# meudnaes/VoronoiRT

Measured on AMD Instinct MI355X. Metric: formal-solve cell-updates/sec, higher is better.
Workload: dtype f64

## Files before the change

### include/voronoirt.h

```cpp
#ifndef VORONOIRT_H
#define VORONOIRT_H

#include <stdint.h>

#ifdef __cplusplus
extern "C" {
#endif

#define VRT_OK 0
#define VRT_EINVAL (-1)
#define VRT_EGRID (-2)
#define VRT_ENODEVICE (-3)
#define VRT_ENOMEM (-4)
#define VRT_EIO (-5)

typedef struct vrt_grid vrt_grid;
typedef struct vrt_plan vrt_plan;

#define VRT_ALPHA_SITE 0
#define VRT_ALPHA_SITE_LAM 1
#define VRT_ALPHA_ANGLE_SITE_LAM 2
#define VRT_ALPHA_ANGLE_NATIVE 3
#define VRT_ALPHA_SITE_LAM_NATIVE 4

// ... 79 lines not shown
int vrt_plan_execute_dev_f32(vrt_plan *p, int64_t nlam, int64_t ld, const float *dS,
                             const float *dalpha, int alpha_mode, const float *dI0_up,
                             const float *dI0_down, const double *weights_host, float *dJ,
                             float *dI_out, void *stream);
int vrt_plan_last_sweep_timing(const vrt_plan *p, double *ms, int64_t *launches);
int vrt_plan_check(vrt_plan *p);
int vrt_plan_last_path(const vrt_plan *p);
int vrt_plan_set_option(vrt_plan *p, const char *name, const char *value);
int vrt_grid_set_option(vrt_grid *g, const char *name, const char *value);

typedef struct vrt_schedule vrt_schedule;
int vrt_schedule_build(const vrt_grid *g, int dir, const int64_t *up, int n_sweeps, vrt_schedule **out);
int64_t vrt_schedule_num_nodes(const vrt_schedule *s);
int64_t vrt_schedule_num_levels(const vrt_schedule *s);
int vrt_schedule_get(const vrt_schedule *s, int64_t *site, int32_t *zflags, int64_t *level_off);
void vrt_schedule_destroy(vrt_schedule *s);
int vrt_layer_schedule(const vrt_grid *g, int dir, const int64_t *up, int n_sweeps, uint32_t *vis,
                       int32_t *nlev, int64_t *n_visits);
int vrt_layer_sorted_slots(const vrt_grid *g, int dir, const uint32_t *vis, int64_t *store, int64_t *self);

typedef struct vrt_patch_schedule vrt_patch_schedule;
int vrt_patch_schedule_build(const vrt_grid *g, int dir, const int64_t *up, int n_sweeps, int own_target,
                             int entry_cap, vrt_patch_schedule **out, int64_t counts[6]);
int vrt_patch_schedule_get(const vrt_patch_schedule *s, int32_t *layer_patch_off, int32_t *patch_own_lo,
                           int32_t *patch_own_cnt, int32_t *patch_nlev, int64_t *patch_ent_off,
                           int32_t *entry_pos, uint32_t *entry_vis, uint32_t *entry_loc);
int vrt_patch_schedule_get_deps(const vrt_patch_schedule *s, int64_t *dep_off, int32_t *dep_list);
int vrt_patch_schedule_get_layers(const vrt_patch_schedule *s, uint32_t *vis, int32_t *nlev, int64_t *n_visits);
void vrt_patch_schedule_destroy(vrt_patch_schedule *s);

int vrt_delaunay_up(vrt_grid *g, const double k[3], const double *S, const double *I0,
                    int64_t nI0, const double *alpha, int n_sweeps, double *I_out);
int vrt_delaunay_down(vrt_grid *g, const double k[3], const double *S, const double *I0,
                      int64_t nI0, const double *alpha, int n_sweeps, double *I_out);

#define VRT_METRIC_EUCLIDEAN   0
#define VRT_METRIC_PERIODIC_XY 1
#define VRT_RASTER_NEAREST     1
#define VRT_RASTER_INV_DIST2   2
int vrt_grid_nearest(vrt_grid *g, int64_t nq, const double *q_zxy, int metric, int k, int64_t *idx, double *dist);
int vrt_grid_to_raster_dev(vrt_grid *g, int64_t nz, int64_t nx, int64_t ny, const double *z, const double *x,
                           const double *y, int metric, int mode, int64_t nf, int64_t ld, const double *d_fields,
                           double *d_raster, void *stream);
int vrt_raster_to_grid_dev(vrt_grid *g, int64_t nz, int64_t nx, int64_t ny, const double *z, const double *x,
                           const double *y, int64_t nf, const double *d_raster, int64_t ld, double *d_fields,
                           void *stream);
// ... 135 lines not shown
```

### voronoirt_amd/_lib.py

```python
from __future__ import annotations

import ctypes
import os

HERE = os.path.dirname(os.path.abspath(__file__))
LIB_PATH = os.path.join(HERE, "libvrt_hip.so")
if os.environ.get("VRT_LIB_PATH"):
    LIB_PATH = os.environ["VRT_LIB_PATH"]

c_i64 = ctypes.c_int64
c_dbl = ctypes.c_double
p_i64 = ctypes.POINTER(ctypes.c_int64)
p_i32 = ctypes.POINTER(ctypes.c_int32)
p_dbl = ctypes.POINTER(ctypes.c_double)
p_int = ctypes.POINTER(ctypes.c_int)
vp = ctypes.c_void_p

VRT_OK, VRT_EINVAL, VRT_EGRID, VRT_ENODEVICE, VRT_ENOMEM, VRT_EIO = 0, -1, -2, -3, -4, -5
ALPHA_SITE, ALPHA_SITE_LAM, ALPHA_ANGLE_SITE_LAM, ALPHA_ANGLE_NATIVE, ALPHA_SITE_LAM_NATIVE = 0, 1, 2, 3, 4
METRIC_EUCLIDEAN, METRIC_PERIODIC_XY = 0, 1
RASTER_NEAREST, RASTER_INV_DIST2 = 1, 2

class LineCaseStruct(ctypes.Structure):
    _fields_ = [("nlam", c_i64), ("lambda_", p_dbl), ("blocks", c_i64 * 6), ("lambda0", c_dbl), ("c0", c_dbl),
# ... 75 lines not shown
                                              p_dbl, p_dbl, p_dbl, p_dbl]),
    "vrt_multi_lambda_create": (ctypes.c_int, [vp, ctypes.POINTER(LineCaseStruct), p_dbl, ctypes.POINTER(vp)]),
    "vrt_multi_lambda_iterate": (ctypes.c_int, [vp, p_dbl]),
    "vrt_multi_lambda_get": (ctypes.c_int, [vp, p_dbl, p_dbl, p_dbl, p_dbl, p_dbl]),
    "vrt_multi_lambda_destroy": (None, [vp]),
    "vrt_rates_populations_dev": (ctypes.c_int, [vp, c_i64, c_i64, p_dbl, p_i64, vp, p_dbl, c_dbl, c_dbl, vp, vp,
                                                 c_dbl, p_dbl, p_dbl, vp, vp, c_dbl, c_dbl, c_dbl, vp, vp, vp,
                                                 vp, vp]),
    "vrt_plan_last_sweep_timing": (ctypes.c_int, [vp, p_dbl, p_i64]),
    "vrt_plan_last_path": (ctypes.c_int, [vp]),
    "vrt_plan_set_option": (ctypes.c_int, [vp, ctypes.c_char_p, ctypes.c_char_p]),
    "vrt_grid_set_option": (ctypes.c_int, [vp, ctypes.c_char_p, ctypes.c_char_p]),
    "vrt_schedule_build": (ctypes.c_int, [vp, ctypes.c_int, p_i64, ctypes.c_int,
                                          ctypes.POINTER(vp)]),
    "vrt_schedule_num_nodes": (c_i64, [vp]),
    "vrt_schedule_num_levels": (c_i64, [vp]),
    "vrt_schedule_get": (ctypes.c_int, [vp, p_i64, p_i32, p_i64]),
    "vrt_schedule_destroy": (None, [vp]),
    "vrt_layer_schedule": (ctypes.c_int, [vp, ctypes.c_int, p_i64, ctypes.c_int,
                                          ctypes.POINTER(ctypes.c_uint32), p_i32, p_i64]),
    "vrt_layer_sorted_slots": (ctypes.c_int, [vp, ctypes.c_int, ctypes.POINTER(ctypes.c_uint32), p_i64, p_i64]),
    "vrt_patch_schedule_build": (ctypes.c_int, [vp, ctypes.c_int, p_i64, ctypes.c_int, ctypes.c_int, ctypes.c_int,
                                                ctypes.POINTER(vp), p_i64]),
    "vrt_patch_schedule_get": (ctypes.c_int, [vp, p_i32, p_i32, p_i32, p_i32, p_i64, p_i32,
                                              ctypes.POINTER(ctypes.c_uint32), ctypes.POINTER(ctypes.c_uint32)]),
    "vrt_patch_schedule_get_deps": (ctypes.c_int, [vp, p_i64, p_i32]),
    "vrt_patch_schedule_get_layers": (ctypes.c_int, [vp, ctypes.POINTER(ctypes.c_uint32), p_i32, p_i64]),
    "vrt_patch_schedule_destroy": (None, [vp]),
    "vrt_lambda_update_dev": (ctypes.c_int, [vp, c_i64, c_i64, vp, vp, vp, vp, vp, p_dbl, vp]),
    "vrt_short_characteristics": (ctypes.c_int, [c_i64, c_i64, c_i64, p_dbl, p_dbl, p_dbl, c_i64, p_dbl,
                                                 p_int, p_dbl, c_i64, p_dbl, c_i64, p_dbl, ctypes.c_int,
                                                 ctypes.c_int, p_dbl]),
    "vrt_regular_create": (ctypes.c_int, [c_i64, c_i64, c_i64, p_dbl, p_dbl, p_dbl, ctypes.c_int,
                                          ctypes.POINTER(vp)]),
    "vrt_regular_destroy": (None, [vp]),
    "vrt_regular_execute_dev": (ctypes.c_int, [vp, c_i64, p_dbl, p_int, vp, c_i64, vp, c_i64, c_i64, vp,
                                               ctypes.c_int, vp, vp]),
    "vrt_regular_last_solve_ms": (ctypes.c_int, [vp, p_dbl]),
    "vrt_synth_opacity_dev": (ctypes.c_int, [c_i64, c_i64, c_i64, p_dbl, c_i64, p_dbl, p_dbl, c_dbl, c_dbl, c_dbl, c_dbl,
                                             c_dbl, c_dbl, c_dbl, c_dbl, vp, vp, vp, vp, vp, vp, vp, vp, vp, vp]),
    "vrt_synth_opacity": (ctypes.c_int, [ctypes.c_int, c_i64, c_i64, c_i64, p_dbl, c_i64, p_dbl, p_dbl, c_dbl, c_dbl,
                                         c_dbl, c_dbl, c_dbl, c_dbl, c_dbl, c_dbl, p_dbl, p_dbl, p_dbl, p_dbl, p_dbl,
                                         p_dbl, p_dbl, p_dbl, p_dbl]),
    "vrt_regular_emergent_dev": (ctypes.c_int, [vp, p_dbl, c_i64, vp, vp, ctypes.c_int, vp, vp]),
    "vrt_top_intensity": (ctypes.c_int, [c_i64, c_i64, c_i64, p_dbl, p_dbl, p_dbl, p_dbl, c_i64, p_dbl, p_dbl,
                                         ctypes.c_int, ctypes.c_int, p_dbl]),
# ... 57 lines not shown
```

### voronoirt_amd/api.py

```python
from __future__ import annotations

import ctypes
import os
import re
import weakref

import numpy as np

from . import _lib
from ._lib import VrtError, check

QUADRATURE_DIR = os.path.join(os.path.dirname(os.path.abspath(__file__)), "quadratures")


def _d(a):
    return a.ctypes.data_as(_lib.p_dbl) if a is not None else None


def _i(a):
    return a.ctypes.data_as(_lib.p_i64) if a is not None else None


def _f64(a):
    return np.ascontiguousarray(a, dtype=np.float64)
# ... 456 lines not shown
        site = np.zeros(nn, dtype=np.int64)
        z = np.zeros(nn, dtype=np.int32)
        off = np.zeros(nl + 1, dtype=np.int64)
        check(L.vrt_schedule_get(h, _i(site), z.ctypes.data_as(_lib.p_i32), _i(off)))
    finally:
        L.vrt_schedule_destroy(h)
    return site, z, off


def build_layer_schedule(sites: VoronoiSites, dir: int, up, n_sweeps: int = 3):
    L = _lib.load()
    up = np.ascontiguousarray(up, dtype=np.int64)
    vis = np.zeros(sites.n, dtype=np.uint32)
    layers = sites.layers_up if dir > 0 else sites.layers_down
    nlev = np.zeros(layers.size, dtype=np.int32)
    nv = ctypes.c_int64()
    check(L.vrt_layer_schedule(sites.handle, int(dir), _i(up), int(n_sweeps),
                               vis.ctypes.data_as(ctypes.POINTER(ctypes.c_uint32)),
                               nlev.ctypes.data_as(_lib.p_i32), ctypes.byref(nv)))
    return vis, nlev, nv.value


def build_patch_schedule(sites: VoronoiSites, dir: int, up, n_sweeps: int = 3, own_target: int = 768,
                         entry_cap: int = 1024) -> dict:
    L = _lib.load()
    up = np.ascontiguousarray(up, dtype=np.int64)
    h = ctypes.c_void_p()
    cnt = np.zeros(6, dtype=np.int64)
    check(L.vrt_patch_schedule_build(sites.handle, int(dir), _i(up), int(n_sweeps), int(own_target), int(entry_cap),
                                     ctypes.byref(h), _i(cnt)))
    try:
        P, E = int(cnt[0]), int(cnt[1])
        out = {"layer_patch_off": np.zeros(int(cnt[5]), dtype=np.int32), "patch_own_lo": np.zeros(P, dtype=np.int32),
               "patch_own_cnt": np.zeros(P, dtype=np.int32), "patch_nlev": np.zeros(P, dtype=np.int32),
               "patch_ent_off": np.zeros(P + 1, dtype=np.int64), "entry_pos": np.zeros(E, dtype=np.int32),
               "entry_vis": np.zeros(E, dtype=np.uint32), "entry_loc": np.zeros(E, dtype=np.uint32)}
        u32 = ctypes.POINTER(ctypes.c_uint32)
        check(L.vrt_patch_schedule_get(h, out["layer_patch_off"].ctypes.data_as(_lib.p_i32),
                                       out["patch_own_lo"].ctypes.data_as(_lib.p_i32),
                                       out["patch_own_cnt"].ctypes.data_as(_lib.p_i32),
                                       out["patch_nlev"].ctypes.data_as(_lib.p_i32), _i(out["patch_ent_off"]),
                                       out["entry_pos"].ctypes.data_as(_lib.p_i32),
                                       out["entry_vis"].ctypes.data_as(u32), out["entry_loc"].ctypes.data_as(u32)))
        out["dep_off"] = np.zeros(P + 1, dtype=np.int64)
        check(L.vrt_patch_schedule_get_deps(h, _i(out["dep_off"]), None))
        out["dep_list"] = np.zeros(int(out["dep_off"][-1]), dtype=np.int32)
        check(L.vrt_patch_schedule_get_deps(h, None, out["dep_list"].ctypes.data_as(_lib.p_i32)))
        out["layer_vis"] = np.zeros(sites.n, dtype=np.uint32)
        out["layer_nlev"] = np.zeros((sites.layers_up if dir > 0 else sites.layers_down).size, dtype=np.int32)
        nv = ctypes.c_int64()
        check(L.vrt_patch_schedule_get_layers(h, out["layer_vis"].ctypes.data_as(u32),
                                              out["layer_nlev"].ctypes.data_as(_lib.p_i32), ctypes.byref(nv)))
        out["layer_visits"] = nv.value
# ... 617 lines not shown
```

### voronoirt_amd/csrc/vrt_api.cpp

```cpp
#include <algorithm>
#include <atomic>
#include <chrono>
#include <cmath>
#include <cstdio>
#include <cstdlib>
#include <cstring>
#include <new>
#include <thread>

#include "vrt_internal.h"

namespace vrt {

static thread_local std::string g_err;

void set_error(const std::string &msg) { g_err = msg; }
int fail(int code, const std::string &msg)
{
    g_err = msg;
    return code;
}

void tuning_from_env(Tuning &t)
{
    static const char *names[] = {"VRT_PATH", "VRT_STEP_K", "VRT_STEP_SINGLE", "VRT_STEP_PAIRS", "VRT_STEP_XCD",
                                  "VRT_STEP_STREAMS", "VRT_STEP_LEVEL_MAP", "VRT_STEP_GROUP_DIR", "VRT_TILE_WIDE",
                                  "VRT_TILE_PRE", "VRT_PATCH_K", "VRT_PATCH_NT", "VRT_PATCH_OWN",
                                  "VRT_PATCH_Q", "VRT_PATCH_TARGET", "VRT_PATCH_SPLIT", "VRT_PAIR_BLOCK", "VRT_PATCH_QUAD", "VRT_PATCH_LEAN", "VRT_PATCH_CHAIN", "VRT_CHAIN_PAIRS", "VRT_CHAIN_SPIN", "VRT_CHAIN_DATAFLAG", "VRT_CHAIN_STATIC", "VRT_LAMBDA_NATIVE", "VRT_DEBUG_FLAGS", "VRT_DEBUG_SKIP_LEVELS",
                                  "VRT_TILE_DEBUG"};
    for (const char *nm : names) {
        const char *e = std::getenv(nm);
        if (e && *e && tuning_set(t, nm, e, false) != VRT_OK) {
            static std::mutex mu;
            static std::vector<std::string> said;
            std::lock_guard<std::mutex> lock(mu);
            if (std::find(said.begin(), said.end(), std::string(nm)) == said.end()) {
                said.push_back(nm);
                std::fprintf(stderr, "[libvrt_hip] ignoring %s=%s: %s\n", nm, e, g_err.c_str());
            }
        }
    }
}

int tuning_set(Tuning &t, const char *name, const char *value, bool created)
{
    if (!name || !value) return fail(VRT_EINVAL, "NULL option name or value");
    const std::string nm(name), v(value);
    if (nm == "VRT_PATH") {
        static const char *paths[] = {"auto", "levels", "tiles", "steps", "patches"};
        for (int i = 0; i < 5; i++)
            if (v == paths[i]) { t.path = i; return VRT_OK; }
        if (v.empty()) { t.path = 0; return VRT_OK; }
        return fail(VRT_EINVAL, "VRT_PATH must be auto, levels, tiles, steps or patches");
    }
    char *end = nullptr;
    const long x = std::strtol(value, &end, 10);
    if (end == value || *end != 0) return fail(VRT_EINVAL, "option " + nm + " needs an integer value");
    struct { const char *name; int *field; long lo, hi; bool creation_only; } tab[] = {
        {"VRT_STEP_K", &t.step_K, 0, 18, false}, {"VRT_STEP_SINGLE", &t.step_single, 0, 1, false},
        {"VRT_STEP_PAIRS", &t.step_pairs, 0, 64, false}, {"VRT_STEP_XCD", &t.step_xcd, 0, 2, false},
        {"VRT_STEP_STREAMS", &t.step_streams, 1, 4, false}, {"VRT_STEP_LEVEL_MAP", &t.step_level_map, 0, 1, false},
        {"VRT_STEP_GROUP_DIR", &t.step_group_dir, 0, 1, false}, {"VRT_TILE_WIDE", &t.tile_wide, 0, 1, false},
        {"VRT_TILE_PRE", &t.tile_pre, 0, 1, false},
        {"VRT_PATCH_K", &t.patch_K, 1, 8, true}, {"VRT_PATCH_NT", &t.patch_NT, 64, 1024, true},
        {"VRT_PATCH_OWN", &t.patch_own, 0, 65535, true}, {"VRT_PATCH_Q", &t.patch_Q, 1, 4, false},
        {"VRT_PATCH_TARGET", &t.patch_target, 0, 1 << 20, false}, {"VRT_PATCH_SPLIT", &t.patch_split, 0, 4096, false}, {"VRT_PAIR_BLOCK", &t.pair_block, 1, 16, true},
        {"VRT_PATCH_QUAD", &t.patch_quad, 0, 1, true}, {"VRT_PATCH_LEAN", &t.patch_lean, 0, 1, false},
        {"VRT_PATCH_CHAIN", &t.patch_chain, 0, 2, false}, {"VRT_CHAIN_PAIRS", &t.chain_pairs, 1, 256, false},
        {"VRT_CHAIN_SPIN", &t.chain_spin, 1, 1 << 20, false}, {"VRT_CHAIN_DATAFLAG", &t.chain_dataflag, 0, 2, false},
        {"VRT_LAMBDA_NATIVE", &t.lambda_native, 0, 1, false}, {"VRT_CHAIN_STATIC", &t.chain_static, 0, 1, false}, {"VRT_DEBUG_FLAGS", &t.debug_flags, 0, 1 << 20, false},
        {"VRT_DEBUG_SKIP_LEVELS", &t.debug_skip_levels, 0, 1, false}, {"VRT_TILE_DEBUG", &t.tile_debug, 0, 1, false},
    };
    for (auto &o : tab)
        if (nm == o.name) {
            if (o.creation_only && created)
                return fail(VRT_EINVAL, "option " + nm + " shapes what plan creation builds: preset it in the environment");
            if (x < o.lo || x > o.hi) return fail(VRT_EINVAL, "option " + nm + " out of range");
            *o.field = (int)x;
            return VRT_OK;
        }
    return fail(VRT_EINVAL, "unknown option " + nm);
}

template <typename T>
static int dev_alloc(T **p, size_t count)
{
    *p = nullptr;
    if (count == 0) count = 1;
// ... 376 lines not shown
            p->tune.patch_K = 1; p->tune.patch_NT = 512; p->tune.patch_Q = 1;
        }
        p->patch_K = p->tune.patch_K;
        p->patch_NT = p->tune.patch_NT;
        p->patch_cap = p->patch_K * p->patch_NT;
        int lg = 0;
        while ((2 << lg) <= p->tune.pair_block && lg < 4) lg++;
        while (lg > 0 && ((uint64_t)n << (lg + 4)) > 0xFFFFFFFFull) lg--;
        p->lg_pair_block = lg;
    }
    const int patch_own = p->tune.patch_own > 0 ? std::min(p->tune.patch_own, p->patch_cap) : p->patch_cap;
    {
        const unsigned hw = std::max(1u, std::thread::hardware_concurrency());
        const int nthr = std::max(1, (int)std::min<unsigned>(std::min(hw, (unsigned)A * 4u <= hw ? 64u : 16u), (unsigned)A));
        const int sub_threads = (int)std::max(1u, std::min(16u, hw / (unsigned)nthr));
        std::atomic<int> next_job(0);
        if (!run_workers(nthr, [&](int) {
                for (;;) {
                    const int a = next_job.fetch_add(1);
                    if (a >= A) break;
                    const bool up = p->dir_of_active[(size_t)a] > 0;
                    const int32_t *u1 = p->h_up1.data() + (size_t)a * n, *u2 = p->h_up2.data() + (size_t)a * n;
                    build_patch_schedule(up ? g->up : g->down, up, n, n_sweeps, u1, u2, patch_own,
                                         p->patch_cap, psched[(size_t)a], sub_threads, &lsched[(size_t)a]);
                    if (!lsched[(size_t)a].ok && lsched[(size_t)a].bad_site < 0)
                        build_layer_schedule(up ? g->up : g->down, up, n, n_sweeps, u1, u2, lsched[(size_t)a]);
                }
            })) {
            free_plan(p);
            return fail(VRT_ENOMEM, "out of host memory while building the sweep schedules");
        }
    }
    tick("layer + patch schedules");
    for (int a = 0; a < A; a++) {
        if (lsched[(size_t)a].bad_site >= 0) {
            std::string msg = "site " + std::to_string(lsched[(size_t)a].bad_site + 1) +
                              " has no neighbour with k . line > -1 for angle " +
                              std::to_string(p->user_of_active[(size_t)a] + 1) +
                              " (the reference reads an uninitialised index here)";
            free_plan(p);
            return fail(VRT_EGRID, msg);
        }
    }
    std::vector<int32_t> ups, downs;
    for (int a = 0; a < A; a++) (p->dir_of_active[(size_t)a] > 0 ? ups : downs).push_back(a);
    p->n_up = (int)ups.size();
    p->n_down = (int)downs.size();
// ... 611 lines not shown
        const int64_t n = g->n;
        const Direction &d = direction_of(g, dir);
        std::vector<uint32_t> v(vis, vis + n);
        std::vector<int32_t> s32;
        build_sorted_slots(d, n, v, s32);
        for (int64_t i = 0; i < n; i++) {
            store[i] = (int64_t)d.store[(size_t)i] + 1;
            self[i] = (int64_t)s32[(size_t)i];
        }
        return VRT_OK;
    } catch (const std::bad_alloc &) {
        return fail(VRT_ENOMEM, "out of host memory");
    }
}

struct vrt_patch_schedule {
    vrt::PatchSchedule s;
    vrt::LayerSchedule layers;
};

int vrt_patch_schedule_build(const vrt_grid *g, int dir, const int64_t *up, int n_sweeps, int own_target,
                             int entry_cap, vrt_patch_schedule **out, int64_t counts[6])
{
    if (!g || !up || !out || !counts) return fail(VRT_EINVAL, "NULL argument");
    if (n_sweeps < 1 || own_target < 1 || entry_cap < 1 || entry_cap > 65535)
        return fail(VRT_EINVAL, "need n_sweeps >= 1, own_target >= 1 and 1 <= entry_cap <= 65535");
    *out = nullptr;
    try {
        const int64_t n = g->n;
        std::vector<int32_t> u1((size_t)n), u2((size_t)n);
        for (int64_t i = 0; i < n; i++) {
            const int64_t a = up[2 * i], b = up[2 * i + 1];
            if (a > n || b > n) return fail(VRT_EINVAL, "upwind id out of range");
            u1[(size_t)i] = a >= 1 ? (int32_t)(a - 1) : kNoUpwind;
            u2[(size_t)i] = b >= 1 ? (int32_t)(b - 1) : kNoUpwind;
        }
        vrt_patch_schedule *ps = new vrt_patch_schedule();
        int threads = (int)std::max(1u, std::min(8u, std::thread::hardware_concurrency()));
        if (const char *e = std::getenv("VRT_HOST_THREADS")) threads = std::max(1, std::min(64, std::atoi(e)));
        build_patch_schedule(direction_of(g, dir), dir > 0, n, n_sweeps, u1.data(), u2.data(), own_target, entry_cap,
                             ps->s, threads, &ps->layers);
        if (ps->s.bad_site >= 0) {
            const std::string msg = "site " + std::to_string(ps->s.bad_site + 1) + " has no upwind neighbour";
            delete ps;
            return fail(VRT_EGRID, msg);
        }
        if (!ps->s.ok) {
            delete ps;
            return fail(VRT_EINVAL, "schedule does not fit the packed patch encoding");
        }
        counts[0] = (int64_t)ps->s.patch_own_lo.size();
        counts[1] = (int64_t)ps->s.entry_pos.size();
        counts[2] = ps->s.n_visits;
        counts[3] = ps->s.n_live;
        counts[4] = ps->s.max_entries;
        counts[5] = (int64_t)ps->s.layer_patch_off.size();
        *out = ps;
        return VRT_OK;
    } catch (const std::bad_alloc &) {
        return fail(VRT_ENOMEM, "out of host memory");
    }
}

int vrt_patch_schedule_get(const vrt_patch_schedule *s, int32_t *layer_patch_off, int32_t *patch_own_lo,
// ... 613 lines not shown
```

### voronoirt_amd/csrc/vrt_grid.cpp

```cpp
#include <algorithm>
#include <cmath>
#include <cstdio>
#include <cstdlib>
#include <cstring>
#include <string>

#include "vrt_internal.h"

namespace vrt {

int parse_neighbour_file(const char *path, int64_t n, std::vector<int64_t> &matrix, int64_t &D1)
{
    FILE *f = std::fopen(path, "rb");
    if (!f) return fail(VRT_EIO, std::string("cannot open neighbour file ") + path);
    std::fseek(f, 0, SEEK_END);
    long sz = std::ftell(f);
    std::fseek(f, 0, SEEK_SET);
    std::vector<char> buf((size_t)sz + 1);
    size_t got = std::fread(buf.data(), 1, (size_t)sz, f);
    std::fclose(f);
    buf[got] = '\n';

    const int64_t cap = kMaxGuess + 1;
    std::vector<int64_t> full((size_t)n * cap, 0);
// ... 116 lines not shown
        for (int64_t i = 0; i < n; i++) {
            double fx = xs > 0 ? (g->pos[3 * (size_t)i + 1] - x0) / xs : 0.0;
            double fy = ys > 0 ? (g->pos[3 * (size_t)i + 2] - y0) / ys : 0.0;
            fx = fx < 0 ? 0 : (fx > 1 ? 1 : fx);
            fy = fy < 0 ? 0 : (fy > 1 ? 1 : fy);
            const uint64_t layer = (uint64_t)(uint32_t)d.layer_of[(size_t)i];
            if (strip_w > 0 && xs > 0 && ys > 0) {
                const double a = cell[(size_t)d.layer_of[(size_t)i]];
                const uint64_t row = std::min<uint64_t>(0x3FFFu, (uint64_t)(fy * ys / (0.5 * a) + 0.25));
                const uint64_t strip = std::min<uint64_t>(0x3FFFu, (uint64_t)(fx * xs / a) / (uint64_t)strip_w);
                key[(size_t)i] = (layer << 42) | (strip << 28) | (row << 14) | (uint64_t)(fx * 16383.0);
                if (i == last_site) key[(size_t)i] = (layer << 42) | 0x3FFFFFFFFFFull;
            } else {
                const uint32_t m = spread((uint32_t)(fx * 65535.0)) | (spread((uint32_t)(fy * 65535.0)) << 1);
                key[(size_t)i] = (layer << 32) | m;
                if (i == last_site) key[(size_t)i] = (layer << 32) | 0xFFFFFFFFull;
            }
        }
        d.store.resize((size_t)n);
        for (int64_t i = 0; i < n; i++) d.store[(size_t)i] = (int32_t)i;
        std::stable_sort(d.store.begin(), d.store.end(), [&](int32_t a, int32_t b) {
            return key[(size_t)a] < key[(size_t)b];
        });
        for (int64_t q = n - 1; q >= 0; q--)
            if (d.store[(size_t)q] == (int32_t)last_site) {
                for (int64_t t = q; t < n - 1; t++) d.store[(size_t)t] = d.store[(size_t)t + 1];
                d.store[(size_t)n - 1] = (int32_t)last_site;
                break;
            }
    }
    return VRT_OK;
}

int build_grid_host(vrt_grid *g, int64_t n, const double *pos, const int64_t *nbr, int64_t D1,
                    const double bounds[6])
{
    if (n < 2 || D1 < 2) return fail(VRT_EINVAL, "grid needs n >= 2 and D1 >= 2");
    if (n >= (int64_t)1 << 30) return fail(VRT_EINVAL, "n must be below 2^30");
    g->n = n;
    std::memcpy(g->bounds, bounds, sizeof(double) * 6);
    g->pos.assign(pos, pos + 3 * n);
    for (int64_t i = 0; i < 3 * n; i++)
        if (!(pos[i] == pos[i])) return fail(VRT_EGRID, "NaN in positions");

    g->rowptr.assign((size_t)n + 1, 0);
    int64_t nnz = 0, D = 0;
// ... 41 lines not shown
```

### voronoirt_amd/csrc/vrt_internal.h

```cpp
#pragma once

#include <hip/hip_runtime.h>

#include <algorithm>
#include <cstdint>
#include <mutex>
#include <string>
#include <thread>
#include <vector>

#include "voronoirt.h"

namespace vrt {

void set_error(const std::string &msg);
int fail(int code, const std::string &msg);

#define VRT_HIP_TRY(expr)                                                                  \
    do {                                                                                   \
        hipError_t _e = (expr);                                                            \
        if (_e != hipSuccess)                                                              \
            return ::vrt::fail(VRT_ENODEVICE, std::string(#expr) + ": " + hipGetErrorString(_e)); \
    } while (0)

// ... 31 lines not shown
        } catch (...) {
            guarded(t);
        }
    }
    for (auto &th : pool) th.join();
    for (int t = 0; t < count; t++)
        if (threw[(size_t)t]) return false;
    return true;
}

constexpr int kMaxAngles = 64;
constexpr int64_t kMaxGuess = 70;
constexpr int32_t kNoUpwind = -1;

struct Direction {
    std::vector<int32_t> layer_of;
    std::vector<int64_t> perm;
    std::vector<int64_t> reduced;
    int64_t n1 = 0;
    int32_t *d_order = nullptr;
    int32_t *d_rank = nullptr;
    int32_t *d_lay = nullptr;
    std::vector<int32_t> store;
    int32_t *d_store = nullptr;
    int32_t *d_srank = nullptr;
};

struct PlanCacheEntry;

struct CopyLane {
    hipStream_t st = nullptr;
    void *pin[2] = {nullptr, nullptr};
    hipEvent_t ev[2] = {nullptr, nullptr};
};
constexpr size_t kCopyChunk = (size_t)8 << 20;

struct Tuning {
    int path = 0;
    int step_K = 0;
    int step_single = 0;
    int step_pairs = 0;
    int step_xcd = 2;
    int step_streams = 2;
    int step_level_map = 1;
    int step_group_dir = 1;
    int tile_wide = 1;
    int tile_pre = 1;
    int patch_K = 1, patch_NT = 512;
    int patch_own = 0;
    int patch_Q = 1;
    int pair_block = 1;
    int patch_quad = 1;
    int patch_lean = 1;
    int patch_chain = 2;
    int chain_pairs = 9;
    int chain_spin = 2048;
    int chain_dataflag = 2;
    int patch_split = 0;
    int patch_target = 0;
    int chain_static = 1;
    int lambda_native = 1;
    int debug_flags = 0, debug_skip_levels = 0, tile_debug = 0;
};
void tuning_from_env(Tuning &t);
int tuning_set(Tuning &t, const char *name, const char *value, bool created);

struct ExecArgs {
    int64_t nlam = 0, ld = 0;
    const void *S = nullptr;
    const void *S_nat[2] = {nullptr, nullptr};
    const void *alpha = nullptr;
    int alpha_mode = 0;
// ... 214 lines not shown
};
void build_layer_schedule(const Direction &dir, bool ascending, int64_t n, int n_sweeps,
                          const int32_t *up1, const int32_t *up2, LayerSchedule &out);
void build_sorted_slots(const Direction &dir, int64_t n, const std::vector<uint32_t> &vis_site,
                        std::vector<int32_t> &self);
struct PatchSchedule {
    std::vector<int32_t> layer_patch_off;
    std::vector<int32_t> patch_own_lo;
    std::vector<int32_t> patch_own_cnt;
    std::vector<int32_t> patch_nlev;
    std::vector<int64_t> patch_ent_off;
    std::vector<int32_t> entry_pos;
    std::vector<uint32_t> entry_vis;
    std::vector<uint32_t> entry_loc;
    std::vector<int64_t> dep_off;
    std::vector<int32_t> dep_list;
    int64_t n_visits = 0;
    int64_t n_live = 0;
    int64_t max_entries = 0;
    int64_t bad_site = -1;
    bool ok = false;
};
void build_patch_schedule(const Direction &dir, bool ascending, int64_t n, int n_sweeps, const int32_t *up1,
                          const int32_t *up2, int own_target, int entry_cap, PatchSchedule &out, int threads = 1,
                          LayerSchedule *layers = nullptr);

int launch_delaunay_lines(vrt_grid *g);
int launch_upwind_table(vrt_plan *p, int a);
struct SweepArgs {
    int64_t n, nlam, ldS, ldA, ldI;
    const void *S, *alpha;
    int alpha_mode;
    void *I;
    bool f32 = false;
};
int launch_boundary(vrt_plan *p, const SweepArgs &sa, const void *dI0_up, const void *dI0_down,
                    hipStream_t st);
int launch_sweep_levels(vrt_plan *p, const SweepArgs &sa, hipStream_t st, int64_t *launches);
int launch_reduce_J(vrt_plan *p, const SweepArgs &sa, const double *weights_active, void *dJ,
                    int64_t ldJ, hipStream_t st);
int launch_copy_I_out(vrt_plan *p, const SweepArgs &sa, void *dI_out, int64_t ldO, hipStream_t st);

int launch_axpy(size_t count, const double *d_src, double *d_dst, hipStream_t st);
int launch_gather_rows(int64_t rows, int64_t nlam, int64_t ld, const int32_t *d_order, const double *d_src, double *d_dst,
                       hipStream_t st);
int launch_lambda_update(int64_t n, int64_t nlam, int64_t ld, const double *dJ, const double *dB,
                         const double *deps, const double *dS_old, double *dS_new,
// ... 65 lines not shown
```

### voronoirt_amd/csrc/vrt_patch.cpp

```cpp
#include <algorithm>
#include <atomic>
#include <new>

#include "vrt_internal.h"

namespace vrt {

namespace {

struct LayerPatches {
    std::vector<int32_t> own_lo, own_cnt, nlev;
    std::vector<int64_t> ent_off;
    std::vector<int32_t> entry_pos;
    std::vector<uint32_t> entry_vis, entry_loc;
    std::vector<uint32_t> vis;
    int32_t layer_nlev = 0;
    int64_t n_visits = 0, n_live = 0, max_entries = 0, bad_site = -1;
    bool ok = true;
    bool levels_ok = false;
};

void build_layer_patches(const Direction &dir, bool ascending, int n_sweeps, const int32_t *up1, const int32_t *up2,
                         int own_target, int entry_cap, int64_t layer, const int32_t *pos_of, LayerPatches &out)
{
    const std::vector<int64_t> &r = dir.reduced;
    const int32_t lo = (int32_t)(r[(size_t)layer - 1] - 1), hi = (int32_t)(r[(size_t)layer] - 1);
    const int32_t m = hi - lo;
    out.ent_off.push_back(0);
    if (m <= 0) return;
    auto local = [&](int32_t site) -> int32_t {
        const int32_t q = pos_of[(size_t)site];
        return dir.layer_of[(size_t)site] == layer && q >= lo && q < hi ? q - lo : -1;
    };
    std::vector<int32_t> l1((size_t)m), l2((size_t)m);
    for (int32_t p = lo; p < hi; p++) {
        const int32_t i = dir.store[(size_t)p];
        const int32_t u1 = up1[i], u2 = up2[i];
        if (u1 < 0 || u2 < 0) {
            if (out.bad_site < 0 || i < out.bad_site) out.bad_site = i;
            l1[(size_t)(p - lo)] = l2[(size_t)(p - lo)] = -1;
            continue;
        }
        l1[(size_t)(p - lo)] = local(u1);
        l2[(size_t)(p - lo)] = local(u2);
    }
    if (out.bad_site >= 0) {
// ... 49 lines not shown
            if (b >= 0) lv = std::max(lv, lw[(size_t)b]);
            lv += 1;
            if (a >= 0) lr[(size_t)a] = std::max(lr[(size_t)a], lv);
            if (b >= 0) lr[(size_t)b] = std::max(lr[(size_t)b], lv);
            lw[li] = lv;
            lr[li] = 0;
            if (lv > 255 || nvis[li] >= 4) {
                out.ok = false;
                return;
            }
            out.vis[li] |= (uint32_t)lv << (8 * nvis[li]);
            nvis[li]++;
            out.n_live++;
            out.layer_nlev = std::max(out.layer_nlev, lv);
        }
        out.levels_ok = true;
    }
    std::vector<int32_t> last_live((size_t)m, -1);
    for (size_t x = 0; x < T; x++)
        if (live[x]) last_live[t_site[x]] = (int32_t)x;
    std::vector<int32_t> stamp(T, -1);
    std::vector<int32_t> slot_of((size_t)m, -1), in_patch((size_t)m, -1);
    std::vector<int32_t> stack, marked, sites, new_marks, new_sites, halo, llw, llr;
    int32_t patch_id = 0;
    int32_t p = 0;
    while (p < m) {
        const int32_t own0 = p;
        marked.clear();
        sites.clear();
        while (p < m && p - own0 < own_target) {
            new_marks.clear();
            new_sites.clear();
            stack.clear();
            const int32_t xs = last_live[(size_t)p];
            if (xs >= 0 && stamp[(size_t)xs] != patch_id) {
                stamp[(size_t)xs] = patch_id;
                stack.push_back(xs);
            }
            while (!stack.empty()) {
                const int32_t x = stack.back();
                stack.pop_back();
                new_marks.push_back(x);
                const int32_t li = (int32_t)t_site[(size_t)x];
                if (in_patch[(size_t)li] != patch_id) {
                    in_patch[(size_t)li] = patch_id;
                    new_sites.push_back(li);
                }
                const int32_t s1 = t_src1[(size_t)x], s2 = t_src2[(size_t)x];
                if (s1 >= 0 && stamp[(size_t)s1] != patch_id) { stamp[(size_t)s1] = patch_id; stack.push_back(s1); }
                if (s2 >= 0 && stamp[(size_t)s2] != patch_id) { stamp[(size_t)s2] = patch_id; stack.push_back(s2); }
            }
            if ((int64_t)sites.size() + (int64_t)new_sites.size() > entry_cap) {
                for (int32_t x : new_marks) stamp[(size_t)x] = -1;
                for (int32_t li : new_sites) in_patch[(size_t)li] = -1;
                break;
            }
            marked.insert(marked.end(), new_marks.begin(), new_marks.end());
            sites.insert(sites.end(), new_sites.begin(), new_sites.end());
            p++;
        }
        const int32_t own_cnt = p - own0;
        if (own_cnt == 0) {
            out.ok = false;
            return;
        }
        halo.clear();
        for (int32_t li : sites)
            if (li < own0 || li >= p) halo.push_back(li);
        std::sort(halo.begin(), halo.end());
        const int64_t entries = (int64_t)own_cnt + (int64_t)halo.size();
        const int64_t e0 = (int64_t)out.entry_pos.size();
        for (int32_t j = 0; j < own_cnt; j++) {
            slot_of[(size_t)(own0 + j)] = j;
            in_patch[(size_t)(own0 + j)] = patch_id;
            out.entry_pos.push_back(lo + own0 + j);
        }
        for (size_t j = 0; j < halo.size(); j++) {
            slot_of[(size_t)halo[j]] = own_cnt + (int32_t)j;
            out.entry_pos.push_back(lo + halo[j]);
        }
        out.entry_vis.resize(out.entry_pos.size(), 0u);
        out.entry_loc.resize(out.entry_pos.size(), 0u);
        std::sort(marked.begin(), marked.end());
        llw.assign((size_t)entries, 0);
        llr.assign((size_t)entries, 0);
        int32_t nlev = 0;
        for (int32_t x : marked) {
            const int32_t li = (int32_t)t_site[(size_t)x];
            const int32_t si = slot_of[(size_t)li];
            const int32_t a = l1[(size_t)li], b = l2[(size_t)li];
            const int32_t c1 = (a >= 0 && in_patch[(size_t)a] == patch_id) ? slot_of[(size_t)a] : -1;
            const int32_t c2 = (b >= 0 && in_patch[(size_t)b] == patch_id) ? slot_of[(size_t)b] : -1;
            int32_t lv = std::max(llw[(size_t)si], llr[(size_t)si]);
            if (c1 >= 0) lv = std::max(lv, llw[(size_t)c1]);
            if (c2 >= 0) lv = std::max(lv, llw[(size_t)c2]);
            lv += 1;
            if (c1 >= 0) llr[(size_t)c1] = std::max(llr[(size_t)c1], lv);
            if (c2 >= 0) llr[(size_t)c2] = std::max(llr[(size_t)c2], lv);
            llw[(size_t)si] = lv;
            llr[(size_t)si] = 0;
            uint32_t &v = out.entry_vis[(size_t)(e0 + si)];
            int sh = 0;
            while (sh < 32 && ((v >> sh) & 0xFFu)) sh += 8;
            v |= (uint32_t)lv << sh;
            nlev = std::max(nlev, lv);
        }
        for (int64_t e = e0; e < (int64_t)out.entry_pos.size(); e++) {
            const int32_t li = out.entry_pos[(size_t)e] - lo;
            uint32_t l[2];
            for (int q = 0; q < 2; q++) {
                const int32_t u = q == 0 ? l1[(size_t)li] : l2[(size_t)li];
                l[q] = (u >= 0 && in_patch[(size_t)u] == patch_id) ? (uint32_t)slot_of[(size_t)u] : 0xFFFFu;
            }
            out.entry_loc[(size_t)e] = l[0] | (l[1] << 16);
        }
        out.own_lo.push_back(lo + own0);
        out.own_cnt.push_back(own_cnt);
        out.nlev.push_back(nlev);
        out.ent_off.push_back((int64_t)out.entry_pos.size());
        out.n_visits += (int64_t)marked.size();
        out.max_entries = std::max<int64_t>(out.max_entries, entries);
        patch_id++;
    }
}

}

void build_patch_schedule(const Direction &dir, bool ascending, int64_t n, int n_sweeps, const int32_t *up1,
                          const int32_t *up2, int own_target, int entry_cap, PatchSchedule &out, int threads,
                          LayerSchedule *layers)
{
    const std::vector<int64_t> &r = dir.reduced;
    const int64_t nl = (int64_t)r.size();
    out = PatchSchedule();
    out.layer_patch_off.assign((size_t)nl + 1, 0);
    out.ok = true;
    if (own_target < 1) own_target = 1;
    if (entry_cap < 1) entry_cap = 1;
    if (entry_cap > 65535) entry_cap = 65535;
    std::vector<int32_t> pos_of((size_t)n);
    for (int64_t p = 0; p < n; p++) pos_of[(size_t)dir.store[(size_t)p]] = (int32_t)p;

    const int64_t first = 2, last = nl - 1;
    const int64_t count = std::max<int64_t>(0, last - first + 1);
    std::vector<LayerPatches> lp((size_t)count);
    std::atomic<int64_t> next(0);
    auto worker = [&](int) {
        for (;;) {
            const int64_t j = next.fetch_add(1);
            if (j >= count) break;
            build_layer_patches(dir, ascending, n_sweeps, up1, up2, own_target, entry_cap, first + j, pos_of.data(), lp[(size_t)j]);
        }
    };
    const int nthr = (int)std::max<int64_t>(1, std::min<int64_t>(threads, count));
    if (nthr <= 1) worker(0);
    else if (!run_workers(nthr, worker)) throw std::bad_alloc();
    for (int64_t j = 0; j < count; j++)
        if (lp[(size_t)j].bad_site >= 0 && (out.bad_site < 0 || lp[(size_t)j].bad_site < out.bad_site)) out.bad_site = lp[(size_t)j].bad_site;
    if (layers) {
        LayerSchedule &ls = *layers;
        ls = LayerSchedule();
        ls.bad_site = out.bad_site;
        ls.nlev.assign((size_t)nl, 0);
        bool all = out.bad_site < 0;
        for (int64_t j = 0; j < count && all; j++) all = lp[(size_t)j].levels_ok || lp[(size_t)j].vis.empty();
        for (int64_t layer = first; layer <= last; layer++)
            ls.max_layer_size = std::max(ls.max_layer_size, r[(size_t)layer] - r[(size_t)layer - 1]);
        if (all) {
            ls.vis.assign((size_t)n, 0u);
            for (int64_t j = 0; j < count; j++) {
                const LayerPatches &l = lp[(size_t)j];
                const int64_t lo = r[(size_t)(first + j) - 1] - 1;
                for (size_t li = 0; li < l.vis.size(); li++) ls.vis[(size_t)dir.store[(size_t)lo + li]] = l.vis[li];
                ls.nlev[(size_t)(first + j)] = l.layer_nlev;
// ... 77 lines not shown
```

Baseline: 88.49 billion.

## Add cone-aware dynamic-programming patch cuts for patch schedules

Replaces the greedy patch partitioning of each layer with a dynamic program. It picks patch boundaries, preferring row starts or fixed strides, so that the patch count is minimised first and the total upwind-cone halo entries second. The aim is fewer patches and less redundant halo recomputation in the patch-based formal solve. This is on by default through a new VRT_PATCH_CUT tuning knob, at the cost of extra host-side schedule build time.

After: 89.32 billion (median of 6 runs). About the same (+0.9%).

```diff
diff --git a/include/voronoirt.h b/include/voronoirt.h
--- a/include/voronoirt.h
+++ b/include/voronoirt.h
@@ -125,6 +125,8 @@
 typedef struct vrt_patch_schedule vrt_patch_schedule;
 int vrt_patch_schedule_build(const vrt_grid *g, int dir, const int64_t *up, int n_sweeps, int own_target,
                              int entry_cap, vrt_patch_schedule **out, int64_t counts[6]);
+int vrt_patch_schedule_build_cut(const vrt_grid *g, int dir, const int64_t *up, int n_sweeps, int own_target,
+                                 int entry_cap, int cut, vrt_patch_schedule **out, int64_t counts[6]);
 int vrt_patch_schedule_get(const vrt_patch_schedule *s, int32_t *layer_patch_off, int32_t *patch_own_lo,
                            int32_t *patch_own_cnt, int32_t *patch_nlev, int64_t *patch_ent_off,
                            int32_t *entry_pos, uint32_t *entry_vis, uint32_t *entry_loc);
diff --git a/voronoirt_amd/_lib.py b/voronoirt_amd/_lib.py
--- a/voronoirt_amd/_lib.py
+++ b/voronoirt_amd/_lib.py
@@ -121,6 +121,8 @@
     "vrt_layer_sorted_slots": (ctypes.c_int, [vp, ctypes.c_int, ctypes.POINTER(ctypes.c_uint32), p_i64, p_i64]),
     "vrt_patch_schedule_build": (ctypes.c_int, [vp, ctypes.c_int, p_i64, ctypes.c_int, ctypes.c_int, ctypes.c_int,
                                                 ctypes.POINTER(vp), p_i64]),
+    "vrt_patch_schedule_build_cut": (ctypes.c_int, [vp, ctypes.c_int, p_i64, ctypes.c_int, ctypes.c_int, ctypes.c_int,
+                                                    ctypes.c_int, ctypes.POINTER(vp), p_i64]),
     "vrt_patch_schedule_get": (ctypes.c_int, [vp, p_i32, p_i32, p_i32, p_i32, p_i64, p_i32,
                                               ctypes.POINTER(ctypes.c_uint32), ctypes.POINTER(ctypes.c_uint32)]),
     "vrt_patch_schedule_get_deps": (ctypes.c_int, [vp, p_i64, p_i32]),
diff --git a/voronoirt_amd/api.py b/voronoirt_amd/api.py
--- a/voronoirt_amd/api.py
+++ b/voronoirt_amd/api.py
@@ -502,13 +502,13 @@
 
 
 def build_patch_schedule(sites: VoronoiSites, dir: int, up, n_sweeps: int = 3, own_target: int = 768,
-                         entry_cap: int = 1024) -> dict:
+                         entry_cap: int = 1024, cut: int = 1) -> dict:
     L = _lib.load()
     up = np.ascontiguousarray(up, dtype=np.int64)
     h = ctypes.c_void_p()
     cnt = np.zeros(6, dtype=np.int64)
-    check(L.vrt_patch_schedule_build(sites.handle, int(dir), _i(up), int(n_sweeps), int(own_target), int(entry_cap),
-                                     ctypes.byref(h), _i(cnt)))
+    check(L.vrt_patch_schedule_build_cut(sites.handle, int(dir), _i(up), int(n_sweeps), int(own_target),
+                                         int(entry_cap), int(cut), ctypes.byref(h), _i(cnt)))
     try:
         P, E = int(cnt[0]), int(cnt[1])
         out = {"layer_patch_off": np.zeros(int(cnt[5]), dtype=np.int32), "patch_own_lo": np.zeros(P, dtype=np.int32),
diff --git a/voronoirt_amd/csrc/vrt_api.cpp b/voronoirt_amd/csrc/vrt_api.cpp
--- a/voronoirt_amd/csrc/vrt_api.cpp
+++ b/voronoirt_amd/csrc/vrt_api.cpp
@@ -25,7 +25,7 @@
 {
     static const char *names[] = {"VRT_PATH", "VRT_STEP_K", "VRT_STEP_SINGLE", "VRT_STEP_PAIRS", "VRT_STEP_XCD",
                                   "VRT_STEP_STREAMS", "VRT_STEP_LEVEL_MAP", "VRT_STEP_GROUP_DIR", "VRT_TILE_WIDE",
-                                  "VRT_TILE_PRE", "VRT_PATCH_K", "VRT_PATCH_NT", "VRT_PATCH_OWN",
+                                  "VRT_TILE_PRE", "VRT_PATCH_K", "VRT_PATCH_NT", "VRT_PATCH_OWN", "VRT_PATCH_CUT",
                                   "VRT_PATCH_Q", "VRT_PATCH_TARGET", "VRT_PATCH_SPLIT", "VRT_PAIR_BLOCK", "VRT_PATCH_QUAD", "VRT_PATCH_LEAN", "VRT_PATCH_CHAIN", "VRT_CHAIN_PAIRS", "VRT_CHAIN_SPIN", "VRT_CHAIN_DATAFLAG", "VRT_CHAIN_STATIC", "VRT_LAMBDA_NATIVE", "VRT_DEBUG_FLAGS", "VRT_DEBUG_SKIP_LEVELS",
                                   "VRT_TILE_DEBUG"};
     for (const char *nm : names) {
@@ -63,7 +63,8 @@
         {"VRT_STEP_GROUP_DIR", &t.step_group_dir, 0, 1, false}, {"VRT_TILE_WIDE", &t.tile_wide, 0, 1, false},
         {"VRT_TILE_PRE", &t.tile_pre, 0, 1, false},
         {"VRT_PATCH_K", &t.patch_K, 1, 8, true}, {"VRT_PATCH_NT", &t.patch_NT, 64, 1024, true},
-        {"VRT_PATCH_OWN", &t.patch_own, 0, 65535, true}, {"VRT_PATCH_Q", &t.patch_Q, 1, 4, false},
+        {"VRT_PATCH_OWN", &t.patch_own, 0, 65535, true}, {"VRT_PATCH_CUT", &t.patch_cut, 0, 1, true},
+        {"VRT_PATCH_Q", &t.patch_Q, 1, 4, false},
         {"VRT_PATCH_TARGET", &t.patch_target, 0, 1 << 20, false}, {"VRT_PATCH_SPLIT", &t.patch_split, 0, 4096, false}, {"VRT_PAIR_BLOCK", &t.pair_block, 1, 16, true},
         {"VRT_PATCH_QUAD", &t.patch_quad, 0, 1, true}, {"VRT_PATCH_LEAN", &t.patch_lean, 0, 1, false},
         {"VRT_PATCH_CHAIN", &t.patch_chain, 0, 2, false}, {"VRT_CHAIN_PAIRS", &t.chain_pairs, 1, 256, false},
@@ -486,7 +487,7 @@
                     const bool up = p->dir_of_active[(size_t)a] > 0;
                     const int32_t *u1 = p->h_up1.data() + (size_t)a * n, *u2 = p->h_up2.data() + (size_t)a * n;
                     build_patch_schedule(up ? g->up : g->down, up, n, n_sweeps, u1, u2, patch_own,
-                                         p->patch_cap, psched[(size_t)a], sub_threads, &lsched[(size_t)a]);
+                                         p->patch_cap, p->tune.patch_cut, psched[(size_t)a], sub_threads, &lsched[(size_t)a]);
                     if (!lsched[(size_t)a].ok && lsched[(size_t)a].bad_site < 0)
                         build_layer_schedule(up ? g->up : g->down, up, n, n_sweeps, u1, u2, lsched[(size_t)a]);
                 }
@@ -1144,7 +1145,14 @@
 int vrt_patch_schedule_build(const vrt_grid *g, int dir, const int64_t *up, int n_sweeps, int own_target,
                              int entry_cap, vrt_patch_schedule **out, int64_t counts[6])
 {
+    return vrt_patch_schedule_build_cut(g, dir, up, n_sweeps, own_target, entry_cap, Tuning().patch_cut, out, counts);
+}
+
+int vrt_patch_schedule_build_cut(const vrt_grid *g, int dir, const int64_t *up, int n_sweeps, int own_target,
+                                 int entry_cap, int cut, vrt_patch_schedule **out, int64_t counts[6])
+{
     if (!g || !up || !out || !counts) return fail(VRT_EINVAL, "NULL argument");
+    if (cut < 0 || cut > 1) return fail(VRT_EINVAL, "cut must be 0 (greedy) or 1 (cone-aware)");
     if (n_sweeps < 1 || own_target < 1 || entry_cap < 1 || entry_cap > 65535)
         return fail(VRT_EINVAL, "need n_sweeps >= 1, own_target >= 1 and 1 <= entry_cap <= 65535");
     *out = nullptr;
@@ -1161,7 +1169,7 @@
         int threads = (int)std::max(1u, std::min(8u, std::thread::hardware_concurrency()));
         if (const char *e = std::getenv("VRT_HOST_THREADS")) threads = std::max(1, std::min(64, std::atoi(e)));
         build_patch_schedule(direction_of(g, dir), dir > 0, n, n_sweeps, u1.data(), u2.data(), own_target, entry_cap,
-                             ps->s, threads, &ps->layers);
+                             cut, ps->s, threads, &ps->layers);
         if (ps->s.bad_site >= 0) {
             const std::string msg = "site " + std::to_string(ps->s.bad_site + 1) + " has no upwind neighbour";
             delete ps;
diff --git a/voronoirt_amd/csrc/vrt_grid.cpp b/voronoirt_amd/csrc/vrt_grid.cpp
--- a/voronoirt_amd/csrc/vrt_grid.cpp
+++ b/voronoirt_amd/csrc/vrt_grid.cpp
@@ -162,6 +162,11 @@
         std::stable_sort(d.store.begin(), d.store.end(), [&](int32_t a, int32_t b) {
             return key[(size_t)a] < key[(size_t)b];
         });
+        if (strip_w > 0 && xs > 0 && ys > 0) {
+            d.row_start.assign((size_t)n, 0);
+            for (int64_t q = 0; q < n; q++)
+                d.row_start[(size_t)q] = q == 0 || (key[(size_t)d.store[(size_t)q]] >> 14) != (key[(size_t)d.store[(size_t)q - 1]] >> 14);
+        }
         for (int64_t q = n - 1; q >= 0; q--)
             if (d.store[(size_t)q] == (int32_t)last_site) {
                 for (int64_t t = q; t < n - 1; t++) d.store[(size_t)t] = d.store[(size_t)t + 1];
diff --git a/voronoirt_amd/csrc/vrt_internal.h b/voronoirt_amd/csrc/vrt_internal.h
--- a/voronoirt_amd/csrc/vrt_internal.h
+++ b/voronoirt_amd/csrc/vrt_internal.h
@@ -77,6 +77,7 @@
     int32_t *d_rank = nullptr;
     int32_t *d_lay = nullptr;
     std::vector<int32_t> store;
+    std::vector<uint8_t> row_start;
     int32_t *d_store = nullptr;
     int32_t *d_srank = nullptr;
 };
@@ -103,6 +104,7 @@
     int tile_pre = 1;
     int patch_K = 1, patch_NT = 512;
     int patch_own = 0;
+    int patch_cut = 1;
     int patch_Q = 1;
     int pair_block = 1;
     int patch_quad = 1;
@@ -363,7 +365,7 @@
     bool ok = false;
 };
 void build_patch_schedule(const Direction &dir, bool ascending, int64_t n, int n_sweeps, const int32_t *up1,
-                          const int32_t *up2, int own_target, int entry_cap, PatchSchedule &out, int threads = 1,
+                          const int32_t *up2, int own_target, int entry_cap, int cut, PatchSchedule &out, int threads = 1,
                           LayerSchedule *layers = nullptr);
 
 int launch_delaunay_lines(vrt_grid *g);
diff --git a/voronoirt_amd/csrc/vrt_patch.cpp b/voronoirt_amd/csrc/vrt_patch.cpp
--- a/voronoirt_amd/csrc/vrt_patch.cpp
+++ b/voronoirt_amd/csrc/vrt_patch.cpp
@@ -7,6 +7,8 @@
 namespace vrt {
 
 namespace {
+
+constexpr int32_t kCutStride = 16;
 
 struct LayerPatches {
     std::vector<int32_t> own_lo, own_cnt, nlev;
@@ -21,7 +23,7 @@
 };
 
 void build_layer_patches(const Direction &dir, bool ascending, int n_sweeps, const int32_t *up1, const int32_t *up2,
-                         int own_target, int entry_cap, int64_t layer, const int32_t *pos_of, LayerPatches &out)
+                         int own_target, int entry_cap, int cut, int64_t layer, const int32_t *pos_of, LayerPatches &out)
 {
     const std::vector<int64_t> &r = dir.reduced;
     const int32_t lo = (int32_t)(r[(size_t)layer - 1] - 1), hi = (int32_t)(r[(size_t)layer] - 1);
@@ -117,47 +119,85 @@
     std::vector<int32_t> stamp(T, -1);
     std::vector<int32_t> slot_of((size_t)m, -1), in_patch((size_t)m, -1);
     std::vector<int32_t> stack, marked, sites, new_marks, new_sites, halo, llw, llr;
-    int32_t patch_id = 0;
-    int32_t p = 0;
-    while (p < m) {
+    int32_t epoch = -1;
+    auto grow = [&](int32_t p) {
+        new_marks.clear();
+        new_sites.clear();
+        stack.clear();
+        const int32_t xs = last_live[(size_t)p];
+        if (xs >= 0 && stamp[(size_t)xs] != epoch) {
+            stamp[(size_t)xs] = epoch;
+            stack.push_back(xs);
+        }
+        while (!stack.empty()) {
+            const int32_t x = stack.back();
+            stack.pop_back();
+            new_marks.push_back(x);
+            const int32_t li = (int32_t)t_site[(size_t)x];
+            if (in_patch[(size_t)li] != epoch) {
+                in_patch[(size_t)li] = epoch;
+                new_sites.push_back(li);
+            }
+            const int32_t s1 = t_src1[(size_t)x], s2 = t_src2[(size_t)x];
+            if (s1 >= 0 && stamp[(size_t)s1] != epoch) { stamp[(size_t)s1] = epoch; stack.push_back(s1); }
+            if (s2 >= 0 && stamp[(size_t)s2] != epoch) { stamp[(size_t)s2] = epoch; stack.push_back(s2); }
+        }
+    };
+    std::vector<int32_t> ends;
+    for (int32_t p = 0; p < m;) {
         const int32_t own0 = p;
+        int64_t cnt = 0;
+        epoch++;
+        while (p < m && p - own0 < own_target) {
+            grow(p);
+            if (cnt + (int64_t)new_sites.size() > entry_cap) break;
+            cnt += (int64_t)new_sites.size();
+            p++;
+        }
+        if (p == own0) {
+            out.ok = false;
+            return;
+        }
+        ends.push_back(p);
+    }
+    if (cut == 1 && ends.size() > 1) {
+        std::vector<uint8_t> cand((size_t)m + 1, 0);
+        const bool rows = !dir.row_start.empty();
+        for (int32_t q = 0; q <= m; q++)
+            cand[(size_t)q] = q == 0 || q == m || (rows ? dir.row_start[(size_t)(lo + q)] != 0 : q % kCutStride == 0);
+        for (int32_t e : ends) cand[(size_t)e] = 1;
+        std::vector<int64_t> best((size_t)m + 1, INT64_MAX);
+        std::vector<int32_t> from((size_t)m + 1, -1);
+        best[0] = 0;
+        for (int32_t s0 = 0; s0 < m; s0++) {
+            if (!cand[(size_t)s0] || best[(size_t)s0] == INT64_MAX) continue;
+            int64_t cnt = 0;
+            epoch++;
+            for (int32_t p = s0; p < m && p - s0 < own_target; p++) {
+                grow(p);
+                cnt += (int64_t)new_sites.size();
+                if (cnt > entry_cap) break;
+                const int64_t c = best[(size_t)s0] + ((int64_t)1 << 32) + cnt;
+                if (cand[(size_t)p + 1] && c < best[(size_t)p + 1]) {
+                    best[(size_t)p + 1] = c;
+                    from[(size_t)p + 1] = s0;
+                }
+            }
+        }
+        ends.clear();
+        for (int32_t q = m; q > 0; q = from[(size_t)q]) ends.push_back(q);
+        std::reverse(ends.begin(), ends.end());
+    }
+    for (size_t k = 0; k < ends.size(); k++) {
+        const int32_t own0 = k == 0 ? 0 : ends[k - 1], p = ends[k];
+        const int32_t own_cnt = p - own0;
         marked.clear();
         sites.clear();
-        while (p < m && p - own0 < own_target) {
-            new_marks.clear();
-            new_sites.clear();
-            stack.clear();
-            const int32_t xs = last_live[(size_t)p];
-            if (xs >= 0 && stamp[(size_t)xs] != patch_id) {
-                stamp[(size_t)xs] = patch_id;
-                stack.push_back(xs);
-            }
-            while (!stack.empty()) {
-                const int32_t x = stack.back();
-                stack.pop_back();
-                new_marks.push_back(x);
-                const int32_t li = (int32_t)t_site[(size_t)x];
-                if (in_patch[(size_t)li] != patch_id) {
-                    in_patch[(size_t)li] = patch_id;
-                    new_sites.push_back(li);
-                }
-                const int32_t s1 = t_src1[(size_t)x], s2 = t_src2[(size_t)x];
-                if (s1 >= 0 && stamp[(size_t)s1] != patch_id) { stamp[(size_t)s1] = patch_id; stack.push_back(s1); }
-                if (s2 >= 0 && stamp[(size_t)s2] != patch_id) { stamp[(size_t)s2] = patch_id; stack.push_back(s2); }
-            }
-            if ((int64_t)sites.size() + (int64_t)new_sites.size() > entry_cap) {
-                for (int32_t x : new_marks) stamp[(size_t)x] = -1;
-                for (int32_t li : new_sites) in_patch[(size_t)li] = -1;
-                break;
-            }
+        epoch++;
+        for (int32_t q = own0; q < p; q++) {
+            grow(q);
             marked.insert(marked.end(), new_marks.begin(), new_marks.end());
             sites.insert(sites.end(), new_sites.begin(), new_sites.end());
-            p++;
-        }
-        const int32_t own_cnt = p - own0;
-        if (own_cnt == 0) {
-            out.ok = false;
-            return;
         }
         halo.clear();
         for (int32_t li : sites)
@@ -167,7 +207,7 @@
         const int64_t e0 = (int64_t)out.entry_pos.size();
         for (int32_t j = 0; j < own_cnt; j++) {
             slot_of[(size_t)(own0 + j)] = j;
-            in_patch[(size_t)(own0 + j)] = patch_id;
+            in_patch[(size_t)(own0 + j)] = epoch;
             out.entry_pos.push_back(lo + own0 + j);
         }
         for (size_t j = 0; j < halo.size(); j++) {
@@ -184,8 +224,8 @@
             const int32_t li = (int32_t)t_site[(size_t)x];
             const int32_t si = slot_of[(size_t)li];
             const int32_t a = l1[(size_t)li], b = l2[(size_t)li];
-            const int32_t c1 = (a >= 0 && in_patch[(size_t)a] == patch_id) ? slot_of[(size_t)a] : -1;
-            const int32_t c2 = (b >= 0 && in_patch[(size_t)b] == patch_id) ? slot_of[(size_t)b] : -1;
+            const int32_t c1 = (a >= 0 && in_patch[(size_t)a] == epoch) ? slot_of[(size_t)a] : -1;
+            const int32_t c2 = (b >= 0 && in_patch[(size_t)b] == epoch) ? slot_of[(size_t)b] : -1;
             int32_t lv = std::max(llw[(size_t)si], llr[(size_t)si]);
             if (c1 >= 0) lv = std::max(lv, llw[(size_t)c1]);
             if (c2 >= 0) lv = std::max(lv, llw[(size_t)c2]);
@@ -205,7 +245,7 @@
             uint32_t l[2];
             for (int q = 0; q < 2; q++) {
                 const int32_t u = q == 0 ? l1[(size_t)li] : l2[(size_t)li];
-                l[q] = (u >= 0 && in_patch[(size_t)u] == patch_id) ? (uint32_t)slot_of[(size_t)u] : 0xFFFFu;
+                l[q] = (u >= 0 && in_patch[(size_t)u] == epoch) ? (uint32_t)slot_of[(size_t)u] : 0xFFFFu;
             }
             out.entry_loc[(size_t)e] = l[0] | (l[1] << 16);
         }
@@ -215,14 +255,13 @@
         out.ent_off.push_back((int64_t)out.entry_pos.size());
         out.n_visits += (int64_t)marked.size();
         out.max_entries = std::max<int64_t>(out.max_entries, entries);
-        patch_id++;
     }
 }
 
 }
 
 void build_patch_schedule(const Direction &dir, bool ascending, int64_t n, int n_sweeps, const int32_t *up1,
-                          const int32_t *up2, int own_target, int entry_cap, PatchSchedule &out, int threads,
+                          const int32_t *up2, int own_target, int entry_cap, int cut, PatchSchedule &out, int threads,
                           LayerSchedule *layers)
 {
     const std::vector<int64_t> &r = dir.reduced;
@@ -244,7 +283,7 @@
         for (;;) {
             const int64_t j = next.fetch_add(1);
             if (j >= count) break;
-            build_layer_patches(dir, ascending, n_sweeps, up1, up2, own_target, entry_cap, first + j, pos_of.data(), lp[(size_t)j]);
+            build_layer_patches(dir, ascending, n_sweeps, up1, up2, own_target, entry_cap, cut, first + j, pos_of.data(), lp[(size_t)j]);
         }
     };
     const int nthr = (int)std::max<int64_t>(1, std::min<int64_t>(threads, count));
```
